# lucastheis/trlda

Hardware: AMD Instinct MI355X
Metric: E-step docs/sec (mini-batch) at K=100, V=7000 (higher is better)
Workload: dtype f64

## Files before the change

trlda_amd/csrc/estep_kernels.h:

```cpp
#pragma once
#include <hip/hip_runtime.h>
#include <stdint.h>

#include <type_traits>

#include "index_params.h"
#include "psi.h"

namespace trlda {

constexpr int kWave = 64;

__device__ __forceinline__ void stores_acknowledged()
{
    asm volatile("s_waitcnt vmcnt(0)" ::: "memory");
    __builtin_amdgcn_fence(__ATOMIC_RELEASE, "workgroup");
}

__device__ __forceinline__ void flag_seen()
{
    __builtin_amdgcn_fence(__ATOMIC_ACQUIRE, "workgroup");
    asm volatile("" ::: "memory");
}

// ... 494 lines not shown
__device__ __forceinline__ void merged_store(double *p, double v, bool coherent)
{
    if (coherent)
        __hip_atomic_store(p, v, __ATOMIC_RELAXED, __HIP_MEMORY_SCOPE_AGENT);
    else
        *p = v;
}

__device__ __forceinline__ double scale_wait_load(const DocKernelArgs &a, int K, int k)
{
    int spins = 0;
    while ((int)(__hip_atomic_load(a.scale_wait + (size_t)doc_block(a) * 16, __ATOMIC_RELAXED,
                                   __HIP_MEMORY_SCOPE_AGENT) - a.epoch) < 0) {
        __builtin_amdgcn_s_sleep(2);
        if (++spins > (1 << 22)) {
            if (a.xerr)
                __hip_atomic_store(a.xerr, 1, __ATOMIC_RELAXED, __HIP_MEMORY_SCOPE_SYSTEM);
            break;
        }
    }
    flag_seen();
    double *in = const_cast<double *>(a.scale_in);
    const double ck = __hip_atomic_load(in + 2 * K + k, __ATOMIC_RELAXED, __HIP_MEMORY_SCOPE_AGENT);
    if (doc_block(a) == 0 && a.scale_out) {
        a.scale_out[k] = __hip_atomic_load(in + k, __ATOMIC_RELAXED, __HIP_MEMORY_SCOPE_AGENT);
        a.scale_out[K + k] = __hip_atomic_load(in + K + k, __ATOMIC_RELAXED, __HIP_MEMORY_SCOPE_AGENT);
        a.scale_out[2 * K + k] = ck;
    }
    return ck;
}

template <int NA>
__device__ __forceinline__ double lds_dot(const double *a, const double *b, int stride, int count)
{
    double acc[NA];
#pragma unroll
    for (int u = 0; u < NA; ++u)
        acc[u] = 0.0;
    int i = 0;
    for (; i + NA <= count; i += NA) {
        double x[NA], y[NA];
#pragma unroll
        for (int u = 0; u < NA; ++u) {
            x[u] = a[i + u];
            y[u] = b[(i + u) * stride];
        }
#pragma unroll
        for (int u = 0; u < NA; ++u)
            acc[u] = fma(x[u], y[u], acc[u]);
    }
#pragma unroll
    for (int u = 0; u < NA - 1; ++u)
        if (i + u < count)
            acc[u] = fma(a[i + u], b[(i + u) * stride], acc[u]);
#pragma unroll
    for (int w = NA / 2; w > 0; w >>= 1)
#pragma unroll
        for (int u = 0; u < w; ++u)
            acc[u] += acc[u + w];
    return acc[0];
}

template <int T>
__device__ __forceinline__ int doc_fixed_point_lds(
    const DocKernelArgs &a, int n, const int32_t *__restrict__ ids,
    const int32_t *__restrict__ cnts, double *__restrict__ beta, double *__restrict__ g,
    double *__restrict__ e, double *__restrict__ tw, double *__restrict__ cntd,
    double *__restrict__ part, double *__restrict__ wsum)
{
    constexpr int W = T / kWave;
    const int tid = threadIdx.x;
    const int lane = tid & (kWave - 1);
    const int wid = tid / kWave;
    const int K = a.K, Kp = a.Kp;

    for (int j = wid; j < n; j += W) {
        const double *src = a.eeb + (size_t)ids[j] * K;
        double *dst = beta + j * Kp;
        for (int k = lane; k < K; k += kWave)
            dst[k] = src[k];
    }
    for (int j = tid; j < n; j += T)
        cntd[j] = (double)cnts[j];

    const int KB = (K + kWave - 1) / kWave;
    const int JP = KB <= W ? W / KB : 1;
    const int JC = (n + JP - 1) / JP;
    const int JB = (n + kWave - 1) / kWave;
    const int KPn = (JB > 0 && JB <= W) ? W / JB : 1;
    const int KC = (K + KPn - 1) / KPn;

    auto product_E = [&]() {
        if (JB <= W) {
            if (wid < JB * KPn) {
                const int jb = wid % JB, kp = wid / JB;
                const int j = jb * kWave + lane;
                const int k0 = kp * KC, k1 = min(K, k0 + KC);
                if (j < n)
                    part[kp * n + j] = lds_dot<8>(e + k0, beta + j * Kp + k0, 1, k1 - k0);
            }
            __syncthreads();
            for (int j = tid; j < n; j += T) {
                double s = part[j];
                for (int q = 1; q < KPn; ++q)
                    s += part[q * n + j];
                tw[j] = cntd[j] / (s + 1e-100);
            }
        } else {
            for (int jb = wid; jb < JB; jb += W) {
                const int j = jb * kWave + lane;
                if (j < n)
                    tw[j] = cntd[j] / (lds_dot<8>(e, beta + j * Kp, 1, K) + 1e-100);
            }
        }
        __syncthreads();
    };

    __syncthreads();
    product_E();

    int it = 0;
    while (it < a.max_iter) {
        if (KB <= W) {
            if (wid < KB * JP) {
                const int kb = wid % KB, jp = wid / KB;
                const int k = kb * kWave + lane;
                const int j0 = min(n, jp * JC), j1 = min(n, j0 + JC);
                if (k < K)
                    part[jp * K + k] = lds_dot<8>(tw + j0, beta + j0 * Kp + k, Kp, j1 - j0);
            }
        } else {
            for (int kb = wid; kb < KB; kb += W) {
                const int k = kb * kWave + lane;
                if (k < K)
                    part[k] = lds_dot<8>(tw, beta + k, Kp, n);
            }
        }
        __syncthreads();

        double diff = 0.0;
        for (int k = tid; k < K; k += T) {
            double acc = part[k];
            for (int q = 1; q < JP; ++q)
                acc += part[q * K + k];
            const double gnew = acc * e[k] + a.alpha[k];
            diff += fabs(g[k] - gnew);
            g[k] = gnew;
            e[k] = exp_digamma(gnew);
        }
        diff = wave_sum(diff);
        if (lane == 0)
            wsum[wid] = diff;
        __syncthreads();

        double change = 0.0;
#pragma unroll
        for (int q = 0; q < W; ++q)
            change += wsum[q];

        product_E();
        ++it;
        if (change / (double)K < a.threshold)
            break;
    }
    return it;
}

template <int T>
__device__ __forceinline__ int doc_fixed_point_stream(
    const DocKernelArgs &a, int n, const int32_t *__restrict__ ids,
    const int32_t *__restrict__ cnts, double *__restrict__ g, double *__restrict__ e,
    double *__restrict__ tw, double *__restrict__ part, double *__restrict__ wsum)
{
    constexpr int W = T / kWave;
    const int tid = threadIdx.x;
    const int lane = tid & (kWave - 1);
    const int wid = tid / kWave;
    const int K = a.K;
    const int kslots = min((K + kWave - 1) / kWave * kWave, T);
    const int jparts = T / kslots;
    const int ks = tid % kslots, jp = tid / kslots;

    auto product_E = [&]() {
        for (int j = wid; j < n; j += W) {
            const double *col = a.eeb + (size_t)ids[j] * K;
            double s = 0.0;
            for (int k = lane; k < K; k += kWave)
                s = fma(e[k], col[k], s);
            s = wave_sum(s);
            if (lane == 0)
                tw[j] = (double)cnts[j] / (s + 1e-100);
        }
        __syncthreads();
    };

    __syncthreads();
    product_E();

    int it = 0;
    while (it < a.max_iter) {
        for (int k = ks; k < K; k += kslots) {
            if (jp < jparts) {
                double acc = 0.0;
                for (int j = jp; j < n; j += jparts)
                    acc = fma(tw[j], a.eeb[(size_t)ids[j] * K + k], acc);
                part[jp * K + k] = acc;
            }
        }
        __syncthreads();
        double diff = 0.0;
        for (int k = tid; k < K; k += T) {
            double acc = part[k];
            for (int q = 1; q < jparts; ++q)
                acc += part[q * K + k];
            const double gnew = acc * e[k] + a.alpha[k];
            diff += fabs(g[k] - gnew);
            g[k] = gnew;
            e[k] = exp_digamma(gnew);
        }
        diff = wave_sum(diff);
        if (lane == 0)
            wsum[wid] = diff;
        __syncthreads();
        double change = 0.0;
#pragma unroll
        for (int q = 0; q < W; ++q)
            change += wsum[q];
        product_E();
        ++it;
        if (change / (double)K < a.threshold)
            break;
    }
    return it;
}

template <int T>
__global__ __launch_bounds__(T) void estep_docs_kernel(DocKernelArgs a)
{
    extern __shared__ double lds[];
    const int tid = threadIdx.x;
    const int lane = tid & (kWave - 1);
    const int wid = tid / kWave;
    constexpr int W = T / kWave;

    const int d = a.order ? a.order[doc_block(a)] : doc_block(a);
    const int K = a.K;
    const int p0 = a.indptr[d];
    const int n = a.indptr[d + 1] - p0;
    const bool staged = n <= a.n_cap;
    const int32_t *ids = a.ids + p0;
    const int32_t *cnts = a.cnts + p0;

    double *beta = lds;
    double *g = beta + a.n_cap * a.Kp;
    double *e = g + K;
    double *tw_l = e + K;
    double *cntd = tw_l + a.n_cap;
    double *part = cntd + a.n_cap;
    double *wsum = part + (K > T ? K : T);

    [[maybe_unused]] unsigned long long stamp_last = 0;
#ifdef TRLDA_STAMPS
    stamp_last = __builtin_amdgcn_s_memtime();
#endif
    double *gamma_d = a.gamma + (size_t)d * K;
    const double *gamma0_d = a.gamma_in + (size_t)d * K;
    for (int k = tid; k < K; k += T) {
        const double gk = gamma0_d[k];
        g[k] = gk;
        e[k] = exp_digamma(gk);
    }

    int it;
    if (staged)
        it = doc_fixed_point_lds<T>(a, n, ids, cnts, beta, g, e, tw_l, cntd, part, wsum);
    else
        it = doc_fixed_point_stream<T>(a, n, ids, cnts, g, e, a.tw_csr + p0, part, wsum);

    for (int k = tid; k < K; k += T) {
        gamma_d[k] = g[k];
        a.epg[(size_t)d * K + k] = e[k];
    }
    if (tid == 0 && a.iters_out)
        a.iters_out[d] = it;

    if (a.sstats_acc) {
        for (int j = wid; j < n; j += W) {
            const double c = staged ? tw_l[j] : a.tw_csr[p0 + j];
            double *col = a.sstats_acc + (size_t)ids[j] * K;
            for (int k = lane; k < K; k += kWave)
                unsafeAtomicAdd(&col[k], c * e[k]);
        }
    } else {
        for (int j = tid; j < n; j += T)
            a.tw_word[a.wrank ? a.wrank[p0 + j] : p0 + j] = staged ? tw_l[j] : a.tw_csr[p0 + j];
    }
}

constexpr int kRegThreads = 512;
constexpr int kRegMaxK = 128;
constexpr int kRegStride = 129;
constexpr int kRegPart = 192;

constexpr int kRegSmallDoubles = 2 * 128 + 2 * 128 + 2 * 144 + 208 + 192 + 8 * kRegPart + 8;
constexpr size_t kRegLdsBytes = (size_t)(kRegSmallDoubles + 128 * kRegStride) * sizeof(double);

template <int CTRL, int ROW_MASK>
__device__ __forceinline__ double dpp_add(double v)
{
    const int lo = __builtin_amdgcn_update_dpp(0, __double2loint(v), CTRL, ROW_MASK, 0xf, false);
    const int hi = __builtin_amdgcn_update_dpp(0, __double2hiint(v), CTRL, ROW_MASK, 0xf, false);
    return v + __hiloint2double(hi, lo);
}
__device__ __forceinline__ double wave_sum_dpp(double v)
{
    v = dpp_add<0x111, 0xf>(v);
    v = dpp_add<0x112, 0xf>(v);
    v = dpp_add<0x114, 0xf>(v);
    v = dpp_add<0x118, 0xf>(v);
    v = dpp_add<0x142, 0xa>(v);
    v = dpp_add<0x143, 0xc>(v);
    const int lo = __builtin_amdgcn_readlane(__double2loint(v), 63);
    const int hi = __builtin_amdgcn_readlane(__double2hiint(v), 63);
    return __hiloint2double(hi, lo);
}

template <int CTRL, int BANK_MASK>
__device__ __forceinline__ double dpp_merge(double old, double src)
{
    const int lo = __builtin_amdgcn_update_dpp(__double2loint(old), __double2loint(src), CTRL, 0xf,
                                               BANK_MASK, false);
    const int hi = __builtin_amdgcn_update_dpp(__double2hiint(old), __double2hiint(src), CTRL, 0xf,
                                               BANK_MASK, false);
    return __hiloint2double(hi, lo);
}

template <int D>
__device__ __forceinline__ double fold(double a, double b)
{
    if constexpr (D == 32) {
        const auto lo = __builtin_amdgcn_permlane32_swap((unsigned)__double2loint(a),
                                                         (unsigned)__double2loint(b), false, false);
        const auto hi = __builtin_amdgcn_permlane32_swap((unsigned)__double2hiint(a),
                                                         (unsigned)__double2hiint(b), false, false);
        return __hiloint2double((int)hi[0], (int)lo[0]) + __hiloint2double((int)hi[1], (int)lo[1]);
    } else if constexpr (D == 16) {
        const auto lo = __builtin_amdgcn_permlane16_swap((unsigned)__double2loint(a),
                                                         (unsigned)__double2loint(b), false, false);
        const auto hi = __builtin_amdgcn_permlane16_swap((unsigned)__double2hiint(a),
                                                         (unsigned)__double2hiint(b), false, false);
        return __hiloint2double((int)hi[0], (int)lo[0]) + __hiloint2double((int)hi[1], (int)lo[1]);
    } else if constexpr (D == 8) {
        const double a2 = dpp_merge<0x128, 0xc>(a, b);
        const double b2 = dpp_merge<0x128, 0x3>(b, a);
        return a2 + b2;
    } else if constexpr (D == 4) {
        const double a2 = dpp_merge<0x114, 0xa>(a, b);
        const double b2 = dpp_merge<0x104, 0x5>(b, a);
        return a2 + b2;
    } else {
        static_assert(D == 2 || D == 1, "fold distance");
        const bool up = (threadIdx.x & D) != 0;
        const double keep = up ? b : a, send = up ? a : b;
        constexpr int CTRL = D == 2 ? 0x4e : 0xb1;
        const int lo = __builtin_amdgcn_update_dpp(0, __double2loint(send), CTRL, 0xf, 0xf, true);
        const int hi = __builtin_amdgcn_update_dpp(0, __double2hiint(send), CTRL, 0xf, 0xf, true);
        return keep + __hiloint2double(hi, lo);
    }
}

template <int N, bool FIRST = false>
__device__ __forceinline__ void fmac_row_bcast(double &acc, double vals, double b)
{
    static_assert(N >= 0 && N < 16, "a lane of the row");
    if constexpr (FIRST)
        asm("s_nop 1\n\tv_fmac_f64_dpp %0, %1, %2 row_newbcast:%3 row_mask:0xf bank_mask:0xf"
            : "+v"(acc)
            : "v"(vals), "v"(b), "n"(N));
    else
        asm("v_fmac_f64_dpp %0, %1, %2 row_newbcast:%3 row_mask:0xf bank_mask:0xf" : "+v"(acc) : "v"(vals), "v"(b), "n"(N));
}
#ifdef TRLDA_WAVE_WEIGHTS
constexpr bool kWaveWeights = true;
#else
constexpr bool kWaveWeights = false;
#endif
#ifndef TRLDA_NO_DPP_BCAST
constexpr bool kDppBcast = true;
#else
constexpr bool kDppBcast = false;
#endif

template <int STRIDE>
__device__ __forceinline__ double sum8_strided(const double *p)
{
    const double v0 = p[0], v1 = p[STRIDE], v2 = p[2 * STRIDE], v3 = p[3 * STRIDE],
                 v4 = p[4 * STRIDE], v5 = p[5 * STRIDE], v6 = p[6 * STRIDE], v7 = p[7 * STRIDE];
    return ((v0 + v1) + (v2 + v3)) + ((v4 + v5) + (v6 + v7));
}

struct PreArgs {
    int n_docs;
    int nb;
    int K, V, G, wpb;
    size_t total;
    const double *lambda;
    double *partial, *u;
    const int32_t *active;
    double *c_out;
    unsigned int *c_counter;
};

template <bool FAT = false, class Pub = NoPublish>
__device__ __forceinline__ void docs_launch_preamble(const PreArgs &pre, double *lds, int block,
                                                     const Pub &pub = Pub(), int tid_bias = 0)
{
    preamble_fused_body<kRegThreads, FAT, Pub>(block - pre.n_docs, pre.nb, lds, pre.K, pre.V, pre.G,
                                     pre.wpb, pre.total, pre.lambda, pre.partial, pre.u, pre.active,
                                     0, nullptr, 0, nullptr, nullptr, pre.c_out, pre.c_counter,
                                     lds + kRegThreads, pub, tid_bias);
}

template <int MODE, bool SPLIT = false>
__device__ __forceinline__ void estep_docs_reg_body(const DocKernelArgs &a, double *lds)
{
    static_assert(MODE == 0 || MODE == 1, "register variants: 128 or 144 words");
    static_assert(!SPLIT || MODE == 0, "segments hold at most 128 words");
    constexpr bool MID = MODE == 1;
    constexpr int JC = MID ? 18 : 16;
    constexpr int NREG = 8 * JC;
    constexpr int T = kRegThreads, W = T / kWave;
    const int tid = threadIdx.x;
    const int lane = tid & (kWave - 1);
    const int wid = __builtin_amdgcn_readfirstlane(tid / kWave);

    const int K = a.K;
    double pv[2][8];
    if (a.partial && !a.scale_in)
        topic_scale_load<T>(K, a.G, a.partial, pv);

    const int bid = doc_block(a);
    const int4 meta = reinterpret_cast<const int4 *>(a.pad_meta)[(size_t)bid * a.meta_i4];
    [[maybe_unused]] int4 seg = make_int4(0, 1, 0, 0);
    if constexpr (SPLIT)
        seg = reinterpret_cast<const int4 *>(a.pad_meta)[(size_t)bid * a.meta_i4 + 1];
    const int32_t *__restrict__ pids = a.pad_ids + (size_t)bid * kRegMaxN;
    const int myid = pids[wid * JC + min(lane, JC - 1)];
    const int d = meta.x, n = meta.y, p0 = meta.z;
    const int32_t *__restrict__ cnts = a.cnts + p0;
    double gk0 = 1.5, ak0 = 0.0, ck0 = 1.0;
    if (tid < K) {
        gk0 = a.gamma_in[(size_t)d * K + tid];
        ak0 = a.alpha[tid];
        if (a.scale_in && !a.scale_wait) {
            ck0 = a.scale_in[2 * K + tid];
            if (bid == 0 && a.scale_out) {
                a.scale_out[tid] = a.scale_in[tid];
                a.scale_out[K + tid] = a.scale_in[K + tid];
                a.scale_out[2 * K + tid] = ck0;
            }
        }
    }

    double *gbuf = lds;
    double *alpha_l = gbuf + 256;
    double *c_l = alpha_l + 128;
    double *ebuf = c_l + 128;
    double *tw = ebuf + 288;
    double *cntd = tw + 208;
    double *part = cntd + 192;
    double *misc = part + 8 * kRegPart;
    double *tbuf = misc + 8;

    [[maybe_unused]] unsigned long long stamp_last = 0;
    TRLDA_STAMP_DECL;
#ifdef TRLDA_STAMPS
    stamp_last = __builtin_amdgcn_s_memtime();
#endif

    const int nm = min(n, NREG);
    const int KC = (((K + W - 1) / W) + 1) & ~1;
    const int j0 = wid * JC, k0 = wid * KC;
    const bool k_lo = lane < K, k_hi = lane + 64 < K;

    double bB0[JC], bB1[JC];
    {
        const int kl = min(lane, K - 1), kh = min(lane + 64, K - 1);
#pragma unroll
        for (int i = 0; i < JC; ++i) {
            const double *rowp = a.eeb + (size_t)__builtin_amdgcn_readlane(myid, i) * K;
            bB0[i] = rowp[kl];
            bB1[i] = rowp[kh];
        }
    }

    [[maybe_unused]] double bE2[4] = {0.0, 0.0, 0.0, 0.0};
    [[maybe_unused]] const int kq = 4 * (lane >> 4);
    if constexpr (MID) {
        const int KCm = (((K + W - 1) / W) + 1) & ~1;
        const int k2 = wid * KCm + kq;
        const int id2 = pids[128 + (lane & 15)];
        const double *row2 = a.eeb + (size_t)id2 * K;
#pragma unroll
        for (int i = 0; i < 4; ++i)
            bE2[i] = row2[min(k2 + i, K - 1)];
    }

    double *gamma_d = a.gamma + (size_t)d * K;
    double e0 = 0.0;
    if (tid < 144) {
        if (tid < K) {
            gbuf[tid] = gk0;
            alpha_l[tid] = ak0;
            e0 = exp_digamma(gk0);
        }
        ebuf[144 + tid] = 0.0;
        if (!a.partial || tid >= K)
            ebuf[tid] = e0;
    }
    if (a.partial && !a.scale_in)
        topic_scale_partials<T>(K, a.G, pv, part);
    for (int j = tid; j < 208; j += T) {
        tw[j] = 0.0;
        if (j < 192)
            cntd[j] = j < n ? (double)cnts[j] : 0.0;
        if (j < 8)
            misc[j] = 0.0;
    }
#pragma unroll
    for (int i = 0; i < JC; ++i) {
        const bool row = j0 + i < nm;
        bB0[i] = (row && k_lo) ? bB0[i] : 0.0;
        bB1[i] = (row && k_hi) ? bB1[i] : 0.0;
    }

#pragma unroll
    for (int i = 0; i < JC; ++i) {
        if (j0 + i < 128) {
            tbuf[(j0 + i) * kRegStride + lane] = bB0[i];
            tbuf[(j0 + i) * kRegStride + 64 + lane] = bB1[i];
        }
    }
    __syncthreads();
    if (tid < K) {
        double ck = 1.0;
        if (a.partial) {
            ck = a.scale_in ? (a.scale_wait ? scale_wait_load(a, K, tid) : ck0)
                            : topic_scale_combine(K, tid, part, a.scale_out);
            ebuf[tid] = e0 * ck;
        }
        c_l[tid] = ck;
    }
    double bE0[16], bE1[16];
    {
        const double *t0 = tbuf + lane * kRegStride + k0;
        const double *t1 = tbuf + (lane + 64) * kRegStride + k0;
        constexpr bool r_lo = true, r_hi = true;
#pragma unroll
        for (int i = 0; i < 16; ++i) {
            const bool colv = i < KC && k0 + i < K;
            const double v0 = t0[colv ? i : 0], v1 = t1[colv ? i : 0];
            bE0[i] = (colv && r_lo) ? v0 : 0.0;
            bE1[i] = (colv && r_hi) ? v1 : 0.0;
        }
    }
    __syncthreads();
    if constexpr (MID) {
        const bool row2_on = 128 + (lane & 15) < nm;
#pragma unroll
        for (int i = 0; i < 4; ++i) {
            const bool colv = kq + i < KC && k0 + kq + i < K;
            bE2[i] = (colv && row2_on) ? bE2[i] : 0.0;
        }
    }
    TRLDA_STAMP(1);
    double *partB = kWaveWeights ? tbuf : part;

    auto product_E = [&](const double *e) {
        const double2 *ep = reinterpret_cast<const double2 *>(e + k0);
        [[maybe_unused]] double2 ew[8];
        [[maybe_unused]] double evals = 0.0, evals2 = 0.0;
        if constexpr (kDppBcast) {
            evals = e[k0 + (lane & 15)];
            if constexpr (MID)
                evals2 = e[k0 + kq + (lane & 3)];
        } else {
#pragma unroll
            for (int i = 0; i < 8; ++i)
                ew[i] = ep[i];
        }
        [[maybe_unused]] double s2 = 0.0;
        if constexpr (MID && kDppBcast) {
            double s2b = 0.0;
            fmac_row_bcast<0, true>(s2, evals2, bE2[0]);
            fmac_row_bcast<1>(s2b, evals2, bE2[1]);
            fmac_row_bcast<2>(s2, evals2, bE2[2]);
            fmac_row_bcast<3>(s2b, evals2, bE2[3]);
            s2 += s2b;
            s2 = fold<32>(s2, s2);
            s2 = fold<16>(s2, s2);
        } else if constexpr (MID) {
#ifndef TRLDA_EXPT_M1_NOS2
            const double2 *eq = reinterpret_cast<const double2 *>(e + k0 + kq);
            const double2 ea = eq[0], eb = eq[1];
            s2 = fma(ea.x, bE2[0], ea.y * bE2[1]) + fma(eb.x, bE2[2], eb.y * bE2[3]);
#ifndef TRLDA_EXPT_M1_NOFOLD
            s2 = fold<32>(s2, s2);
            s2 = fold<16>(s2, s2);
#endif
#endif
        }
        double s0[4] = {0.0, 0.0, 0.0, 0.0}, s1[4] = {0.0, 0.0, 0.0, 0.0};
        if constexpr (kDppBcast) {
#define TRLDA_E_STEP(t, F)                                       \
    fmac_row_bcast<t, F>(s0[(t) & 3], evals, bE0[t]);            \
    fmac_row_bcast<t>(s1[(t) & 3], evals, bE1[t]);
            TRLDA_E_STEP(0, true) TRLDA_E_STEP(1, false) TRLDA_E_STEP(2, false) TRLDA_E_STEP(3, false)
            TRLDA_E_STEP(4, false) TRLDA_E_STEP(5, false) TRLDA_E_STEP(6, false) TRLDA_E_STEP(7, false)
            TRLDA_E_STEP(8, false) TRLDA_E_STEP(9, false) TRLDA_E_STEP(10, false) TRLDA_E_STEP(11, false)
            TRLDA_E_STEP(12, false) TRLDA_E_STEP(13, false) TRLDA_E_STEP(14, false) TRLDA_E_STEP(15, false)
#undef TRLDA_E_STEP
        } else {
#pragma unroll
            for (int i = 0; i < 8; ++i) {
                s0[(2 * i) & 3] = fma(ew[i].x, bE0[2 * i], s0[(2 * i) & 3]);
                s1[(2 * i) & 3] = fma(ew[i].x, bE1[2 * i], s1[(2 * i) & 3]);
                s0[(2 * i + 1) & 3] = fma(ew[i].y, bE0[2 * i + 1], s0[(2 * i + 1) & 3]);
                s1[(2 * i + 1) & 3] = fma(ew[i].y, bE1[2 * i + 1], s1[(2 * i + 1) & 3]);
            }
        }
        part[wid * kRegPart + lane] = (s0[0] + s0[1]) + (s0[2] + s0[3]);
        part[wid * kRegPart + 64 + lane] = (s1[0] + s1[1]) + (s1[2] + s1[3]);
        if constexpr (MID) {
            if (lane < 16)
                part[wid * kRegPart + 128 + lane] = s2;
        }
        __syncthreads();
        if constexpr (!kWaveWeights) {
            if (tid < 128 || tid < n)
                tw[tid] = cntd[tid] * rcp_pos<true>(sum8_strided<kRegPart>(part + tid) + 1e-100);
            __syncthreads();
        }
    };
    auto wave_weights = [&]() {
        const int jl = j0 + (MID ? min(lane, JC - 1) : (lane & 15));
        if constexpr (!kWaveWeights)
            return tw[jl];
        return cntd[jl] * rcp_pos<true>(sum8_strided<kRegPart>(part + jl) + 1e-100);
    };

    product_E(ebuf);
    TRLDA_STAMP(2);

    const int k_psi = (wid & 1) * 64 + lane;
    const bool psi_on = k_psi < K;
    const double c_psi = c_l[psi_on ? k_psi : 0];

    const double thresholdK = a.threshold * (double)K;
    int it = 0;
    while (it < a.max_iter) {
        {
            double a0[4] = {0.0, 0.0, 0.0, 0.0}, a1[4] = {0.0, 0.0, 0.0, 0.0};
            const double tvals_w = wave_weights();
#ifdef TRLDA_M1_DPP_B
            constexpr bool dpp_b = kDppBcast;
#else
            constexpr bool dpp_b = kDppBcast && !MID;
#endif
            if constexpr (dpp_b) {
                const double tvals = MID ? tw[j0 + min(lane & 15, JC - 1)] : tvals_w;
                [[maybe_unused]] double tvals2 = 0.0;
                if constexpr (MID)
                    tvals2 = tw[j0 + 16 + (lane & 1)];
#define TRLDA_B_STEP(w, F)                                       \
    fmac_row_bcast<w, F>(a0[(w) & 3], tvals, bB0[w]);            \
    fmac_row_bcast<w>(a1[(w) & 3], tvals, bB1[w]);
                TRLDA_B_STEP(0, true) TRLDA_B_STEP(1, false) TRLDA_B_STEP(2, false) TRLDA_B_STEP(3, false)
                TRLDA_B_STEP(4, false) TRLDA_B_STEP(5, false) TRLDA_B_STEP(6, false) TRLDA_B_STEP(7, false)
                TRLDA_B_STEP(8, false) TRLDA_B_STEP(9, false) TRLDA_B_STEP(10, false) TRLDA_B_STEP(11, false)
                TRLDA_B_STEP(12, false) TRLDA_B_STEP(13, false) TRLDA_B_STEP(14, false) TRLDA_B_STEP(15, false)
#undef TRLDA_B_STEP
                if constexpr (MID) {
                    fmac_row_bcast<0, true>(a0[0], tvals2, bB0[16]);
                    fmac_row_bcast<0>(a1[0], tvals2, bB1[16]);
                    fmac_row_bcast<1>(a0[1], tvals2, bB0[17]);
                    fmac_row_bcast<1>(a1[1], tvals2, bB1[17]);
                }
            } else {
                if constexpr (kWaveWeights) {
                    if (lane < JC)
                        tw[j0 + lane] = tvals_w;
                    __builtin_amdgcn_fence(__ATOMIC_RELEASE, "wavefront");
                    __builtin_amdgcn_wave_barrier();
                }
                const double2 *tp = reinterpret_cast<const double2 *>(tw + j0);
                double2 tv[JC / 2];
#pragma unroll
                for (int i = 0; i < JC / 2; ++i)
                    tv[i] = tp[i];
#pragma unroll
                for (int i = 0; i < JC / 2; ++i) {
                    a0[(2 * i) & 3] = fma(tv[i].x, bB0[2 * i], a0[(2 * i) & 3]);
                    a1[(2 * i) & 3] = fma(tv[i].x, bB1[2 * i], a1[(2 * i) & 3]);
                    a0[(2 * i + 1) & 3] = fma(tv[i].y, bB0[2 * i + 1], a0[(2 * i + 1) & 3]);
                    a1[(2 * i + 1) & 3] = fma(tv[i].y, bB1[2 * i + 1], a1[(2 * i + 1) & 3]);
                }
            }
            partB[wid * kRegPart + lane] = (a0[0] + a0[1]) + (a0[2] + a0[3]);
            partB[wid * kRegPart + 64 + lane] = (a1[0] + a1[1]) + (a1[2] + a1[3]);
        }
        __syncthreads();
        TRLDA_STAMP(3);

        const double *g_old = gbuf + (it & 1) * 128, *e_old = ebuf + (it & 1) * 144;
        double *g_new = gbuf + ((it + 1) & 1) * 128, *e_new = ebuf + ((it + 1) & 1) * 144;
        if (wid < 2) {
            const int kk = psi_on ? k_psi : 0;
            const double ek = e_old[kk], ak = alpha_l[kk];
            double acc = sum8_strided<kRegPart>(partB + kk);
            if constexpr (SPLIT) {
                double *rows = a.xbuf + ((size_t)seg.z * (size_t)(a.max_iter + 1) +
                                         (size_t)it * (size_t)seg.y) * (size_t)K;
                if (psi_on)
                    __hip_atomic_store(rows + (size_t)seg.x * K + k_psi,
                                       acc == acc ? acc : __longlong_as_double(0x7FF8000000000000ll),
                                       __ATOMIC_RELAXED, __HIP_MEMORY_SCOPE_AGENT);
                double total = 0.0;
                for (int c0 = 0; c0 < seg.y; c0 += 8) {
                    double v[8];
                    const int nc = min(8, seg.y - c0);
                    unsigned need = (1u << nc) - 1u;
                    for (int spins = 0;; ++spins) {
#pragma unroll
                        for (int c = 0; c < 8; ++c)
                            if (need >> c & 1u)
                                v[c] = __hip_atomic_load(rows + (size_t)(c0 + c) * K + kk, __ATOMIC_RELAXED,
                                                         __HIP_MEMORY_SCOPE_AGENT);
                        unsigned still = 0u;
#pragma unroll
                        for (int c = 0; c < 8; ++c)
                            if ((need >> c & 1u) && __double_as_longlong(v[c]) == -1ll)
                                still |= 1u << c;
                        need = still;
                        if (!__any(need != 0u))
                            break;
                        const bool lost = spins > (1 << 21) ||
                                          ((spins & 1023) == 1023 &&
                                           __hip_atomic_load(a.xerr, __ATOMIC_RELAXED, __HIP_MEMORY_SCOPE_SYSTEM) != 0);
                        if (lost) {
                            if (lane == 0) {
                                __hip_atomic_store(a.xerr, 1, __ATOMIC_RELAXED, __HIP_MEMORY_SCOPE_SYSTEM);
                                misc[2 + wid] = 1.0;
                            }
#pragma unroll
                            for (int c = 0; c < 8; ++c)
                                if (need >> c & 1u)
                                    v[c] = 0.0;
                            break;
                        }
                    }
#pragma unroll
                    for (int c = 0; c < 8; ++c)
                        if (c < nc)
                            total += v[c];
                }
                acc = total;
            }
            const double gnew = acc * ek + ak;
            const double enew = exp_digamma(gnew) * c_psi;
            if (psi_on) {
                g_new[k_psi] = gnew;
                e_new[k_psi] = enew;
            }
            if constexpr (SPLIT) {
                const double half = wave_sum_dpp(psi_on ? fabs(g_old[kk] - gnew) : 0.0);
                if (lane == 0)
                    misc[wid] = half;
            }
        } else if (!SPLIT && wid >= W - 2) {
            const int kc = (wid - (W - 2)) * 64 + lane;
            const bool on = kc < K;
            const int ka = on ? kc : 0;
            const double *pp = partB + ka;
            const double p0v = pp[0], p1v = pp[kRegPart], p2v = pp[2 * kRegPart], p3v = pp[3 * kRegPart],
                         p4v = pp[4 * kRegPart], p5v = pp[5 * kRegPart], p6v = pp[6 * kRegPart],
                         p7v = pp[7 * kRegPart];
            const double eo = e_old[ka], al = alpha_l[ka], go = g_old[ka];
            __builtin_amdgcn_sched_barrier(0);
            const double ga = (((p0v + p1v) + (p2v + p3v)) + ((p4v + p5v) + (p6v + p7v))) * eo + al;
            const double v = on ? fabs(go - ga) : 0.0;
            const double half = wave_sum_dpp(v);
            if (lane == 0)
                misc[wid - (W - 2)] = half;
        }
        TRLDA_STAMP(7);
        __syncthreads();
        TRLDA_STAMP(4);
        const double change_sum = misc[0] + misc[1];
        if constexpr (SPLIT) {
            if (misc[2] + misc[3] != 0.0)
                break;
        }

        product_E(e_new);
        TRLDA_STAMP(5);
        ++it;
        if (change_sum < thresholdK)
            break;
    }
    const double *g = gbuf + (it & 1) * 128, *e = ebuf + (it & 1) * 144;
    if constexpr (kWaveWeights) {
        if (tid < 128 || tid < n)
            tw[tid] = cntd[tid] * rcp_pos<true>(sum8_strided<kRegPart>(part + tid) + 1e-100);
        __syncthreads();
    }

    if (!SPLIT || seg.x == 0) {
        for (int k = tid; k < K; k += T) {
            gamma_d[k] = g[k];
            merged_store(a.epg + (size_t)d * K + k, e[k], a.done_counter != nullptr);
        }
        if (tid == 0 && a.iters_out)
            a.iters_out[d] = it;
    }
    if (a.sstats_acc) {
        for (int j = wid; j < n; j += W) {
            const double c = tw[j];
            double *col = a.sstats_acc + (size_t)pids[j] * K;
            for (int k = lane; k < K; k += kWave)
                unsafeAtomicAdd(&col[k], c * e[k]);
        }
    } else {
        if (tid < n)
            merged_store(a.tw_word + (a.wrank ? a.wrank[p0 + tid] : p0 + tid), tw[tid],
                         a.done_counter != nullptr);
    }
    TRLDA_STAMP(6);
    TRLDA_STAMP_FLUSH;
}

__device__ __forceinline__ void estep_docs_small_body(const DocKernelArgs &a, double *lds)
{
    constexpr int T = kRegThreads, KM = 32;
    const int tid = threadIdx.x;
    const int lane = tid & (kWave - 1);
    const int wid = __builtin_amdgcn_readfirstlane(tid / kWave);
    const int K = a.K;
    double pv[2][8];
    if (a.partial && !a.scale_in)
        topic_scale_load<T>(K, a.G, a.partial, pv);

    const int bid = doc_block(a);
    const int di = a.small_first + (bid - a.small_block0) * 8 + wid;
    const bool doc_on = di < a.B;
    const int dc = min(di, a.B - 1);
    int4 meta;
    int id0, id1;
    if (a.meta_i4 == 2) {
        const int dd = a.order[dc];
        const int q0 = a.indptr[dd], nn = a.indptr[dd + 1] - q0;
        meta = make_int4(dd, nn, q0, 0);
        id0 = a.ids[q0 + min(lane, max(nn - 1, 0))];
        id1 = a.ids[q0 + min(lane + 64, max(nn - 1, 0))];
        if (nn == 0)
            id0 = id1 = 0;
    } else {
        meta = reinterpret_cast<const int4 *>(a.pad_meta)[dc];
        const int32_t *__restrict__ pids = a.pad_ids + (size_t)dc * kRegMaxN;
        id0 = pids[lane];
        id1 = pids[64 + lane];
    }
    const int d = meta.x, n = doc_on ? meta.y : 0, p0 = meta.z;
    const int kt = lane >> 1;
    const bool k_on = kt < K;
    const int kc = k_on ? kt : 0;
    double g = a.gamma_in[(size_t)d * K + kc];
    const double ak = a.alpha[kc];
    const double cnt0 = lane < n ? (double)a.cnts[p0 + lane] : 0.0;
    const double cnt1 = lane + 64 < n ? (double)a.cnts[p0 + 64 + lane] : 0.0;
    double ck0 = 1.0;
    if (tid < K && a.scale_in && !a.scale_wait) {
        ck0 = a.scale_in[2 * K + tid];
        if (bid == 0 && a.scale_out) {
            a.scale_out[tid] = a.scale_in[tid];
            a.scale_out[K + tid] = a.scale_in[K + tid];
            a.scale_out[2 * K + tid] = ck0;
        }
    }
    double u0[KM], u1[KM];
    {
        const double *r0 = a.eeb + (size_t)id0 * K, *r1 = a.eeb + (size_t)id1 * K;
        const bool on0 = lane < n, on1 = lane + 64 < n;
        const bool k_even = (K & 1) == 0;
#pragma unroll
        for (int k = 0; k < KM; k += 2) {
            double2 v0 = make_double2(0.0, 0.0), v1 = make_double2(0.0, 0.0);
            if (k < K && k_even) {
                v0 = *reinterpret_cast<const double2 *>(r0 + k);
                v1 = *reinterpret_cast<const double2 *>(r1 + k);
            } else if (k < K) {
                v0.x = r0[k];
                v1.x = r1[k];
                if (k + 1 < K) {
                    v0.y = r0[k + 1];
                    v1.y = r1[k + 1];
                }
            }
            u0[k] = on0 ? v0.x : 0.0; u0[k + 1] = on0 ? v0.y : 0.0;
            u1[k] = on1 ? v1.x : 0.0; u1[k + 1] = on1 ? v1.y : 0.0;
        }
    }
    double *part = lds, *c_l = lds + 8 * 128;
    if (a.partial && !a.scale_in)
        topic_scale_partials<T>(K, a.G, pv, part);
    __syncthreads();
    if (tid < K) {
        double ck = 1.0;
        if (a.partial)
            ck = a.scale_in ? (a.scale_wait ? scale_wait_load(a, K, tid) : ck0)
                            : topic_scale_combine(K, tid, part, a.scale_out);
        c_l[tid] = ck;
    }
    __syncthreads();
    if (!doc_on)
        return;
    const double ck = c_l[kc];
    double e = k_on ? exp_digamma(g) * ck : 0.0;
    const int elo0 = 0;
    (void)elo0;
    double tw0 = 0.0, tw1 = 0.0;
    auto weights = [&]() {
        const int lo = __double2loint(e), hi = __double2hiint(e);
        double s0[2] = {0.0, 0.0}, s1[2] = {0.0, 0.0};
#pragma unroll
        for (int k = 0; k < KM; ++k) {
            if (k < K) {
                const double ek = __hiloint2double(__builtin_amdgcn_readlane(hi, 2 * k),
                                                   __builtin_amdgcn_readlane(lo, 2 * k));
                s0[k & 1] = fma(ek, u0[k], s0[k & 1]);
                s1[k & 1] = fma(ek, u1[k], s1[k & 1]);
            }
        }
        tw0 = cnt0 * rcp_pos<true>((s0[0] + s0[1]) + 1e-100);
        tw1 = cnt1 * rcp_pos<true>((s1[0] + s1[1]) + 1e-100);
    };
    weights();
    const double thresholdK = a.threshold * (double)K;
    int it = 0;
    while (it < a.max_iter) {
        double q16[16], q8[8], q4[4], q2[2];
#pragma unroll
        for (int i = 0; i < 16; ++i) {
            const double pa = i < K ? fma(tw1, u1[i], tw0 * u0[i]) : 0.0;
            const double pb = i + 16 < K ? fma(tw1, u1[i + 16], tw0 * u0[i + 16]) : 0.0;
            q16[i] = fold<32>(pa, pb);
        }
#pragma unroll
        for (int i = 0; i < 8; ++i)
            q8[i] = fold<16>(q16[i], q16[i + 8]);
#pragma unroll
        for (int i = 0; i < 4; ++i)
            q4[i] = fold<8>(q8[i], q8[i + 4]);
        q2[0] = fold<4>(q4[0], q4[2]);
        q2[1] = fold<4>(q4[1], q4[3]);
        const double q1 = fold<2>(q2[0], q2[1]);
        const double acc = fold<1>(q1, q1);
        const double gnew = acc * e + ak;
        const double enew = k_on ? exp_digamma(gnew) * ck : 0.0;
        const double change_sum = wave_sum_dpp((k_on && !(lane & 1)) ? fabs(g - gnew) : 0.0);
        g = gnew;
        e = enew;
        weights();
        ++it;
        if (change_sum < thresholdK)
            break;
    }
    if (k_on && !(lane & 1)) {
        a.gamma[(size_t)d * K + kt] = g;
        merged_store(a.epg + (size_t)d * K + kt, e, a.done_counter != nullptr);
    }
    if (lane == 0 && a.iters_out)
        a.iters_out[d] = it;
    if (lane < n)
        merged_store(a.tw_word + (a.wrank ? a.wrank[p0 + lane] : p0 + lane), tw0, a.done_counter != nullptr);
    if (lane + 64 < n)
        merged_store(a.tw_word + (a.wrank ? a.wrank[p0 + 64 + lane] : p0 + 64 + lane), tw1,
                     a.done_counter != nullptr);
}

template <int MODE>
__global__ __launch_bounds__(kRegThreads) void estep_docs_reg_kernel(DocKernelArgs a, PreArgs pre)
{
    extern __shared__ __attribute__((aligned(16))) double lds[];
    if ((int)blockIdx.x >= pre.n_docs) {
        docs_launch_preamble(pre, lds, (int)blockIdx.x);
        return;
    }
    if (a.docs_per_wg == 8)
        estep_docs_small_body(a, lds);
    else
        estep_docs_reg_body<MODE>(a, lds);
}

struct TwView {
    const double *v;
    const int32_t *idx;
    __device__ __forceinline__ double operator[](int q) const { return idx ? v[idx[q]] : v[q]; }
};

#ifndef TRLDA_STAT_ROWS
#define TRLDA_STAT_ROWS 4
#endif
#ifndef TRLDA_STAT_ROWS2
#define TRLDA_STAT_ROWS2 4
#endif
constexpr int kStatRows = TRLDA_STAT_ROWS;
constexpr int kStatRows2 = TRLDA_STAT_ROWS2;

template <int NH>
__device__ __forceinline__ void word_segment_sum(int q0, int q1, int K, int kbase,
                                                 const int32_t *__restrict__ wdoc,
                                                 TwView tw_word,
                                                 const double *__restrict__ epg, double *acc)
{
    const int lane = threadIdx.x & (kWave - 1);
    int kk[NH];
#pragma unroll
    for (int h = 0; h < NH; ++h)
        kk[h] = min(kbase + 64 * h + lane, K - 1);
    int dl = lane < q1 - q0 ? wdoc[q0 + lane] : 0;
    double tl = lane < q1 - q0 ? tw_word[q0 + lane] : 0.0;
    for (int q = q0; q < q1; q += 16) {
        const int cnt = min(16, q1 - q);
        const int dcur = dl;
        const int tlo = __double2loint(tl), thi = __double2hiint(tl);
        if (q + 16 < q1) {
            const bool more = lane < q1 - q - 16;
            dl = more ? wdoc[q + 16 + lane] : 0;
            tl = more ? tw_word[q + 16 + lane] : 0.0;
        }
#pragma unroll
        for (int grp = 0; grp < 16 / kStatRows; ++grp) {
            if (kStatRows * grp < cnt) {
                double ev[kStatRows][NH];
#pragma unroll
                for (int u = 0; u < kStatRows; ++u) {
                    const size_t row = (size_t)__builtin_amdgcn_readlane(dcur, kStatRows * grp + u) * K;
#pragma unroll
                    for (int h = 0; h < NH; ++h)
                        ev[u][h] = epg[row + kk[h]];
                }
#pragma unroll
                for (int u = 0; u < kStatRows; ++u) {
                    const double tu =
                        __hiloint2double(__builtin_amdgcn_readlane(thi, kStatRows * grp + u),
                                         __builtin_amdgcn_readlane(tlo, kStatRows * grp + u));
#pragma unroll
                    for (int h = 0; h < NH; ++h)
                        acc[h] = fma(tu, ev[u][h], acc[h]);
                }
            }
        }
    }
}


struct VeryLongArgs {
    int G_seg;
    int seg_len;
    int n_tasks, n_words;
    const int4 *task;
    const int4 *word;
    int j0, t0;
    double *seg_partial;
    unsigned int *seg_counter;
    int row_base;
    int n_rows;
};

__device__ __forceinline__ int long_first_block(int G_short, int long_len)
{
    if (long_len <= kLongWord)
        return (int)blockIdx.x;
    const int nb = (int)gridDim.x;
    const int b = (int)blockIdx.x + G_short;
    return b >= nb ? b - nb : b;
}

template <int T>
__global__ __launch_bounds__(T) void sstats_words_kernel(
    int K, int V, int G_short, int long_len, const int32_t *__restrict__ wptr,
    const int32_t *__restrict__ wdoc, const int32_t *__restrict__ long_words, TwView tw_word,
    const double *__restrict__ epg, const double *__restrict__ eeb, double *__restrict__ sstats)
{
    constexpr int W = T / kWave;
    extern __shared__ double wpart[];
    const int lane = threadIdx.x & (kWave - 1);
    const int wid = __builtin_amdgcn_readfirstlane(threadIdx.x / kWave);
    const int bid = long_first_block(G_short, long_len);

    if (bid < G_short) {
        const int w = wid * G_short + bid;
        if (w >= V)
            return;
        const int q0 = __builtin_amdgcn_readfirstlane(wptr[w]);
        const int len = __builtin_amdgcn_readfirstlane(wptr[w + 1]) - q0;
        if (len > long_len)
            return;
        for (int kb = 0; kb < K; kb += 2 * kWave) {
            double acc[2] = {0.0, 0.0};
            if (len > 0)
                word_segment_sum<2>(q0, q0 + len, K, kb, wdoc, tw_word, epg, acc);
#pragma unroll
            for (int h = 0; h < 2; ++h) {
                const int k = kb + 64 * h + lane;
                if (k < K) {
                    const size_t i = (size_t)w * K + k;
                    sstats[i] = len > 0 ? acc[h] * eeb[i] : 0.0;
                }
            }
        }
        return;
    }

    const int w = long_words[bid - G_short];
    const int base = __builtin_amdgcn_readfirstlane(wptr[w]);
    const int L = __builtin_amdgcn_readfirstlane(wptr[w + 1]) - base;
    const int chunk = (L + W - 1) / W;
    const int c0 = __builtin_amdgcn_readfirstlane(min(L, wid * chunk));
    const int c1 = __builtin_amdgcn_readfirstlane(min(L, c0 + chunk));
    for (int kb = 0; kb < K; kb += 2 * kWave) {
        double acc[2] = {0.0, 0.0};
        word_segment_sum<2>(base + c0, base + c1, K, kb, wdoc, tw_word, epg, acc);
#pragma unroll
        for (int h = 0; h < 2; ++h) {
            const int k = kb + 64 * h + lane;
            if (k < K)
// ... 589 lines not shown
```

Baseline: 7.481 million.

## Size register E-step DPP loops to actual word and topic counts

Result: faster. 7.675 million, median of 5 (+2.6%).

```diff
diff --git a/trlda_amd/csrc/estep_kernels.h b/trlda_amd/csrc/estep_kernels.h
--- a/trlda_amd/csrc/estep_kernels.h
+++ b/trlda_amd/csrc/estep_kernels.h
@@ -820,7 +820,7 @@
 constexpr int kRegStride = 129;
 constexpr int kRegPart = 192;
 
-constexpr int kRegSmallDoubles = 2 * 128 + 2 * 128 + 2 * 144 + 208 + 192 + 8 * kRegPart + 8;
+constexpr int kRegSmallDoubles = 2 * 128 + 2 * 128 + 2 * 144 + 208 + 192 + 8 * kRegPart + 8 + 96;
 constexpr size_t kRegLdsBytes = (size_t)(kRegSmallDoubles + 128 * kRegStride) * sizeof(double);
 
 template <int CTRL, int ROW_MASK>
@@ -903,6 +903,27 @@
 #else
 constexpr bool kWaveWeights = false;
 #endif
+#ifndef TRLDA_NO_SIZED_BODY
+constexpr bool kSizedBody = true;
+#else
+constexpr bool kSizedBody = false;
+#endif
+#ifndef TRLDA_SIZED_PIECES
+#define TRLDA_SIZED_PIECES 14
+#endif
+constexpr int kSizedPieces = TRLDA_SIZED_PIECES;
+#define TRLDA_STEPS_SIZED(S, cnt)                                                        \
+    S(0, true) S(1, false) S(2, false) S(3, false) S(4, false) S(5, false) S(6, false)   \
+    S(7, false) S(8, false) S(9, false) S(10, false) S(11, false) S(12, false)           \
+    if ((cnt) > 13) {                                                                    \
+        S(13, false)                                                                     \
+        if ((cnt) > 14) {                                                                \
+            S(14, false)                                                                 \
+            if ((cnt) > 15) {                                                            \
+                S(15, false)                                                             \
+            }                                                                            \
+        }                                                                                \
+    }
 #ifndef TRLDA_NO_DPP_BCAST
 constexpr bool kDppBcast = true;
 #else
@@ -947,6 +968,8 @@
     constexpr bool MID = MODE == 1;
     constexpr int JC = MID ? 18 : 16;
     constexpr int NREG = 8 * JC;
+    constexpr bool SIZED = kSizedBody && !MID && kDppBcast;
+    constexpr bool DEALT = SIZED && (kSizedPieces & 16);
     constexpr int T = kRegThreads, W = T / kWave;
     const int tid = threadIdx.x;
     const int lane = tid & (kWave - 1);
@@ -963,7 +986,7 @@
     if constexpr (SPLIT)
         seg = reinterpret_cast<const int4 *>(a.pad_meta)[(size_t)bid * a.meta_i4 + 1];
     const int32_t *__restrict__ pids = a.pad_ids + (size_t)bid * kRegMaxN;
-    const int myid = pids[wid * JC + min(lane, JC - 1)];
+    const int myid = pids[DEALT ? 8 * min(lane, JC - 1) + wid : wid * JC + min(lane, JC - 1)];
     const int d = meta.x, n = meta.y, p0 = meta.z;
     const int32_t *__restrict__ cnts = a.cnts + p0;
     double gk0 = 1.5, ak0 = 0.0, ck0 = 1.0;
@@ -988,7 +1011,8 @@
     double *cntd = tw + 208;
     double *part = cntd + 192;
     double *misc = part + 8 * kRegPart;
-    double *tbuf = misc + 8;
+    int *wrk = reinterpret_cast<int *>(misc + 8);
+    double *tbuf = misc + 8 + 96;
 
     [[maybe_unused]] unsigned long long stamp_last = 0;
     TRLDA_STAMP_DECL;
@@ -997,8 +1021,16 @@
 #endif
 
     const int nm = min(n, NREG);
-    const int KC = (((K + W - 1) / W) + 1) & ~1;
+    const int KC = SIZED && (kSizedPieces & 2) ? (K + W - 1) / W : (((K + W - 1) / W) + 1) & ~1;
     const int j0 = wid * JC, k0 = wid * KC;
+    const int jc = __builtin_amdgcn_readfirstlane((nm + W - 1) / W);
+    const int b_steps = DEALT && (kSizedPieces & 1) ? jc : 16;
+    const int e_steps = SIZED && (kSizedPieces & 2) ? KC : 16;
+    constexpr bool STAGE_ROWS = DEALT && (kSizedPieces & 4), STAGE_COLS = SIZED && (kSizedPieces & 4);
+    constexpr bool TAIL_EARLY = SIZED && (kSizedPieces & 8);
+    auto word_of = [&](int i) { return DEALT ? 8 * i + wid : j0 + i; };
+    auto row_on = [&](int i) { return !STAGE_ROWS || i < 13 || i < jc; };
+    auto col_on = [&](int i) { return !STAGE_COLS || i < 13 || i < KC; };
     const bool k_lo = lane < K, k_hi = lane + 64 < K;
 
     double bB0[JC], bB1[JC];
@@ -1006,9 +1038,12 @@
         const int kl = min(lane, K - 1), kh = min(lane + 64, K - 1);
 #pragma unroll
         for (int i = 0; i < JC; ++i) {
-            const double *rowp = a.eeb + (size_t)__builtin_amdgcn_readlane(myid, i) * K;
-            bB0[i] = rowp[kl];
-            bB1[i] = rowp[kh];
+            bB0[i] = bB1[i] = 0.0;
+            if (row_on(i)) {
+                const double *rowp = a.eeb + (size_t)__builtin_amdgcn_readlane(myid, i) * K;
+                bB0[i] = rowp[kl];
+                bB1[i] = rowp[kh];
+            }
         }
     }
 
@@ -1040,23 +1075,26 @@
         topic_scale_partials<T>(K, a.G, pv, part);
     for (int j = tid; j < 208; j += T) {
         tw[j] = 0.0;
-        if (j < 192)
+        if (j < 192) {
             cntd[j] = j < n ? (double)cnts[j] : 0.0;
+            if constexpr (TAIL_EARLY)
+                wrk[j] = j < n ? (a.wrank ? a.wrank[p0 + j] : p0 + j) : 0;
+        }
         if (j < 8)
             misc[j] = 0.0;
     }
 #pragma unroll
     for (int i = 0; i < JC; ++i) {
-        const bool row = j0 + i < nm;
+        const bool row = word_of(i) < nm;
         bB0[i] = (row && k_lo) ? bB0[i] : 0.0;
         bB1[i] = (row && k_hi) ? bB1[i] : 0.0;
     }
 
 #pragma unroll
     for (int i = 0; i < JC; ++i) {
-        if (j0 + i < 128) {
-            tbuf[(j0 + i) * kRegStride + lane] = bB0[i];
-            tbuf[(j0 + i) * kRegStride + 64 + lane] = bB1[i];
+        if (word_of(i) < 128 && row_on(i)) {
+            tbuf[word_of(i) * kRegStride + lane] = bB0[i];
+            tbuf[word_of(i) * kRegStride + 64 + lane] = bB1[i];
         }
     }
     __syncthreads();
@@ -1073,13 +1111,16 @@
     {
         const double *t0 = tbuf + lane * kRegStride + k0;
         const double *t1 = tbuf + (lane + 64) * kRegStride + k0;
-        constexpr bool r_lo = true, r_hi = true;
+        const bool r_lo = !STAGE_ROWS || lane < nm, r_hi = !STAGE_ROWS || lane + 64 < nm;
 #pragma unroll
         for (int i = 0; i < 16; ++i) {
-            const bool colv = i < KC && k0 + i < K;
-            const double v0 = t0[colv ? i : 0], v1 = t1[colv ? i : 0];
-            bE0[i] = (colv && r_lo) ? v0 : 0.0;
-            bE1[i] = (colv && r_hi) ? v1 : 0.0;
+            bE0[i] = bE1[i] = 0.0;
+            if (col_on(i)) {
+                const bool colv = i < KC && k0 + i < K;
+                const double v0 = t0[colv ? i : 0], v1 = t1[colv ? i : 0];
+                bE0[i] = (colv && r_lo) ? v0 : 0.0;
+                bE1[i] = (colv && r_hi) ? v1 : 0.0;
+            }
         }
     }
     __syncthreads();
@@ -1133,10 +1174,7 @@
 #define TRLDA_E_STEP(t, F)                                       \
     fmac_row_bcast<t, F>(s0[(t) & 3], evals, bE0[t]);            \
     fmac_row_bcast<t>(s1[(t) & 3], evals, bE1[t]);
-            TRLDA_E_STEP(0, true) TRLDA_E_STEP(1, false) TRLDA_E_STEP(2, false) TRLDA_E_STEP(3, false)
-            TRLDA_E_STEP(4, false) TRLDA_E_STEP(5, false) TRLDA_E_STEP(6, false) TRLDA_E_STEP(7, false)
-            TRLDA_E_STEP(8, false) TRLDA_E_STEP(9, false) TRLDA_E_STEP(10, false) TRLDA_E_STEP(11, false)
-            TRLDA_E_STEP(12, false) TRLDA_E_STEP(13, false) TRLDA_E_STEP(14, false) TRLDA_E_STEP(15, false)
+            TRLDA_STEPS_SIZED(TRLDA_E_STEP, e_steps)
 #undef TRLDA_E_STEP
         } else {
 #pragma unroll
@@ -1161,7 +1199,7 @@
         }
     };
     auto wave_weights = [&]() {
-        const int jl = j0 + (MID ? min(lane, JC - 1) : (lane & 15));
+        const int jl = MID ? j0 + min(lane, JC - 1) : word_of(lane & 15);
         if constexpr (!kWaveWeights)
             return tw[jl];
         return cntd[jl] * rcp_pos<true>(sum8_strided<kRegPart>(part + jl) + 1e-100);
@@ -1193,10 +1231,7 @@
 #define TRLDA_B_STEP(w, F)                                       \
     fmac_row_bcast<w, F>(a0[(w) & 3], tvals, bB0[w]);            \
     fmac_row_bcast<w>(a1[(w) & 3], tvals, bB1[w]);
-                TRLDA_B_STEP(0, true) TRLDA_B_STEP(1, false) TRLDA_B_STEP(2, false) TRLDA_B_STEP(3, false)
-                TRLDA_B_STEP(4, false) TRLDA_B_STEP(5, false) TRLDA_B_STEP(6, false) TRLDA_B_STEP(7, false)
-                TRLDA_B_STEP(8, false) TRLDA_B_STEP(9, false) TRLDA_B_STEP(10, false) TRLDA_B_STEP(11, false)
-                TRLDA_B_STEP(12, false) TRLDA_B_STEP(13, false) TRLDA_B_STEP(14, false) TRLDA_B_STEP(15, false)
+                TRLDA_STEPS_SIZED(TRLDA_B_STEP, b_steps)
 #undef TRLDA_B_STEP
                 if constexpr (MID) {
                     fmac_row_bcast<0, true>(a0[0], tvals2, bB0[16]);
@@ -1350,7 +1385,7 @@
         }
     } else {
         if (tid < n)
-            merged_store(a.tw_word + (a.wrank ? a.wrank[p0 + tid] : p0 + tid), tw[tid],
+            merged_store(a.tw_word + (TAIL_EARLY ? wrk[tid] : a.wrank ? a.wrank[p0 + tid] : p0 + tid), tw[tid],
                          a.done_counter != nullptr);
     }
     TRLDA_STAMP(6);
```
